# 12334zq/optical-flow-1

Hardware: AMD Instinct MI355X
Metric: Mpix*warp-iters/s, TV-L1 1920x1080 5-scale (higher is better)
Workload: dtype f64; 1 GPU; tvl1flow 1920x1080 pair (synthetic P1), nscales=5 warps=5 tau=0.25 lambda=0.15 theta=0.3 zfactor=0.5 epsilon=0.01; one pair per step per GPU; workload_name=1080p, arithmetic_mode=tolerance, pairs_per_gpu=1040, pairs_in_flight_per_gpu=64, lockstep_group=16, streams_per_gpu=4, distinct_pairs=8

## Files before the change

optical-flow-1_amd/csrc/ofx_device.h:

```cpp
#pragma once

#include <hip/hip_runtime.h>

#define OFX_DEV __device__ __forceinline__

OFX_DEV double  ldw(const double *p) { return *p; }
OFX_DEV double  ldw(const float *p)  { return (double) *p; }
OFX_DEV double2 ldw2(const double2 *p) { return *p; }
OFX_DEV double2 ldw2(const float2 *p)  { float2 v = *p; return make_double2((double) v.x, (double) v.y); }
OFX_DEV double4 ldw4(const double4 *p) { return *p; }
OFX_DEV double4 ldw4(const float4 *p)
{
    float4 v = *p;
    return make_double4((double) v.x, (double) v.y, (double) v.z, (double) v.w);
}
OFX_DEV void stn(double *p, double v) { *p = v; }
OFX_DEV void stn(float *p, double v)  { *p = (float) v; }
OFX_DEV void stn2(double2 *p, double2 v) { *p = v; }
OFX_DEV void stn2(float2 *p, double2 v)  { *p = make_float2((float) v.x, (float) v.y); }
typedef double ofx_d2v __attribute__((ext_vector_type(2)));
typedef float ofx_f2v __attribute__((ext_vector_type(2)));
OFX_DEV void stn2_nt(double2 *p, double2 v)
{
    ofx_d2v w;
    w.x = v.x; w.y = v.y;
    __builtin_nontemporal_store(w, reinterpret_cast<ofx_d2v *>(p));
}
OFX_DEV void stn2_nt(float2 *p, double2 v)
{
    ofx_f2v w;
    w.x = (float) v.x; w.y = (float) v.y;
    __builtin_nontemporal_store(w, reinterpret_cast<ofx_f2v *>(p));
}
template <bool NT, typename V> OFX_DEV void stn2_sel(V *p, double2 v)
{
    if (NT) stn2_nt(p, v);
    else stn2(p, v);
}
#define OFX_OOB 0xFFFFFFF0u
typedef unsigned ofx_u4v __attribute__((ext_vector_type(4)));
typedef unsigned ofx_u2v __attribute__((ext_vector_type(2)));
typedef __amdgpu_buffer_rsrc_t ofx_rsrc;
OFX_DEV ofx_rsrc make_rsrc(void *p, unsigned bytes) { return __builtin_amdgcn_make_buffer_rsrc(p, 0, bytes, 0x00020000); }
template <bool NT> OFX_DEV void bst2(ofx_rsrc r, unsigned byte_off, double2 v, const double2 *)
{
    ofx_u4v w;
    __builtin_memcpy(&w, &v, 16);
    __builtin_amdgcn_raw_buffer_store_b128(w, r, byte_off, 0, NT ? 2 : 0);
}
template <bool NT> OFX_DEV void bst2(ofx_rsrc r, unsigned byte_off, double2 v, const float2 *)
{
    const float2 f = make_float2((float) v.x, (float) v.y);
// ... 209 lines not shown
    }
    return cubic_cell(c[0], c[1], c[2], c[3], t.fx);
}

template <typename V2, typename S>
OFX_DEV void bicubic_sample3(const V2 *__restrict__ pa, const S *__restrict__ pb, const BicubicTaps &t, int nx,
                             double &o0, double &o1, double &o2)
{
    const unsigned E = sizeof(S);
    const unsigned r0 = (unsigned) t.row[0] * nx * E, r1 = (unsigned) t.row[1] * nx * E;
    const unsigned r2 = (unsigned) t.row[2] * nx * E, r3 = (unsigned) t.row[3] * nx * E;
    double c0[4], c1[4], c2[4];
#pragma unroll
    for (int k = 0; k < 4; k++) {
        const unsigned ck = (unsigned) t.col[k] * E;
        const char *ba = reinterpret_cast<const char *>(pa), *bb = reinterpret_cast<const char *>(pb);
        const double2 a0 = ldw2(reinterpret_cast<const V2 *>(ba + 2 * (r0 + ck)));
        const double2 a1 = ldw2(reinterpret_cast<const V2 *>(ba + 2 * (r1 + ck)));
        const double2 a2 = ldw2(reinterpret_cast<const V2 *>(ba + 2 * (r2 + ck)));
        const double2 a3 = ldw2(reinterpret_cast<const V2 *>(ba + 2 * (r3 + ck)));
        const double b0 = ldw(reinterpret_cast<const S *>(bb + r0 + ck));
        const double b1 = ldw(reinterpret_cast<const S *>(bb + r1 + ck));
        const double b2 = ldw(reinterpret_cast<const S *>(bb + r2 + ck));
        const double b3 = ldw(reinterpret_cast<const S *>(bb + r3 + ck));
        c0[k] = cubic_cell(a0.x, a1.x, a2.x, a3.x, t.fy);
        c1[k] = cubic_cell(a0.y, a1.y, a2.y, a3.y, t.fy);
        c2[k] = cubic_cell(b0, b1, b2, b3, t.fy);
    }
    o0 = cubic_cell(c0[0], c0[1], c0[2], c0[3], t.fx);
    o1 = cubic_cell(c1[0], c1[1], c1[2], c1[3], t.fx);
    o2 = cubic_cell(c2[0], c2[1], c2[2], c2[3], t.fx);
}

OFX_DEV double div_backward(double ac, double al, double bc, double bu, bool lef, bool rig, bool top, bool bot)
{
    if (!lef && !rig) {
        const double dxv = ac - al;
        return top ? dxv + bc : (bot ? dxv - bu : dxv + (bc - bu));
    }
    if (lef) return top ? ac + bc : (bot ? ac - bu : ac + bc - bu);
    return top ? -al + bc : (bot ? -al - bu : -al + bc - bu);
}
```

optical-flow-1_amd/csrc/ofx_ops.hip:

```cpp
#include "ofx_ops.h"
#include "ofx_device.h"

#include <cmath>

#define BX 64
#define BY 4

static inline dim3 grid2d(int nx, int ny) { return dim3(ofx_cdiv(nx, BX), ofx_cdiv(ny, BY)); }
static inline dim3 block2d() { return dim3(BX, BY); }
static inline int grid1d(size_t n) { return (int) ((n + 255) / 256); }

template <typename T>
__global__ void k_convert_in(const double *__restrict__ src, T *__restrict__ dst, size_t n)
{
    const size_t i = (size_t) blockIdx.x * blockDim.x + threadIdx.x;
    if (i < n) stn(dst + i, src[i]);
}

template <typename T>
__global__ void k_convert_out(const T *__restrict__ src, double *__restrict__ dst, size_t n)
{
    const size_t i = (size_t) blockIdx.x * blockDim.x + threadIdx.x;
    if (i < n) dst[i] = ldw(src + i);
}
// ... 253 lines not shown
    __shared__ double s_mid[(GXY_TH + 2 * GXY_RMAX) * 64];
    const T *__restrict__ in = in_p.at(blockIdx.z);
    T *__restrict__ out = out_p.at(blockIdx.z);
    const int R = taps.size - 1, W = 64 + 2 * R, H = GXY_TH + 2 * R;
    const int j0 = blockIdx.x * 64, i0 = blockIdx.y * GXY_TH;
    const int tid = threadIdx.y * 64 + threadIdx.x;
    for (int k = tid; k < W * H; k += 256) {
        const int r = k / W, c = k - r * W;
        int i = gauss_reflect(i0 - R + r, ny), j = gauss_reflect(j0 - R + c, nx);
        i = i < 0 ? 0 : (i > ny - 1 ? ny - 1 : i);
        j = j < 0 ? 0 : (j > nx - 1 ? nx - 1 : j);
        s_in[r * W + c] = ldw(in + (size_t) i * nx + j);
    }
    __syncthreads();
    for (int r = threadIdx.y; r < H; r += 4) {
        const double *row = s_in + r * W + R + threadIdx.x;
        double sum = taps.B[0] * row[0];
        for (int k = 1; k < taps.size; k++) sum += taps.B[k] * (row[-k] + row[k]);
        s_mid[r * 64 + threadIdx.x] = sizeof(T) == sizeof(float) ? (double) (float) sum : sum;
    }
    __syncthreads();
    const int j = j0 + threadIdx.x;
    if (j >= nx) return;
    for (int r = threadIdx.y; r < GXY_TH; r += 4) {
        const int i = i0 + r;
        if (i >= ny) break;
        const double *col = s_mid + (r + R) * 64 + threadIdx.x;
        double sum = taps.B[0] * col[0];
        for (int k = 1; k < taps.size; k++) sum += taps.B[k] * (col[-k * 64] + col[k * 64]);
        stn(out + (size_t) i * nx + j, sum);
    }
}

template <typename T, int R>
__global__ __launch_bounds__(256) void k_gauss_xy_gr(OfxPlanes2<const T> in_p, OfxPlanes2<T> out_p, int nx, int ny, GaussTaps taps)
{
    constexpr int W = 64 + 2 * R, H = GXY_TH + 2 * R;
    __shared__ double s_in[H * W];
    __shared__ double s_mid[H * 64];
    const T *__restrict__ in = in_p.at(blockIdx.z);
    T *__restrict__ out = out_p.at(blockIdx.z);
    const int j0 = blockIdx.x * 64, i0 = blockIdx.y * GXY_TH;
    const int tx = threadIdx.x, ty = threadIdx.y;
    int ja = gauss_reflect(j0 - R + tx, nx), jb = gauss_reflect(j0 - R + tx + 64, nx);
    ja = ja < 0 ? 0 : (ja > nx - 1 ? nx - 1 : ja);
    jb = jb < 0 ? 0 : (jb > nx - 1 ? nx - 1 : jb);
    for (int r = ty; r < H; r += 4) {
        int i = gauss_reflect(i0 - R + r, ny);
        i = i < 0 ? 0 : (i > ny - 1 ? ny - 1 : i);
        const T *__restrict__ row = in + (size_t) i * nx;
        s_in[r * W + tx] = ldw(row + ja);
        if (tx < 2 * R) s_in[r * W + tx + 64] = ldw(row + jb);
    }
    __syncthreads();
    for (int r = ty; r < H; r += 4) {
        const double *row = s_in + r * W + R + tx;
        double sum = taps.B[0] * row[0];
#pragma unroll
        for (int k = 1; k <= R; k++) sum += taps.B[k] * (row[-k] + row[k]);
        s_mid[r * 64 + tx] = sizeof(T) == sizeof(float) ? (double) (float) sum : sum;
    }
    __syncthreads();
    const int j = j0 + tx;
    if (j >= nx) return;
    constexpr int SEG = GXY_TH / 4;
    double win[SEG + 2 * R];
#pragma unroll
    for (int q = 0; q < SEG + 2 * R; q++) win[q] = s_mid[(ty * SEG + q) * 64 + tx];
#pragma unroll
    for (int o = 0; o < SEG; o++) {
        const int i = i0 + ty * SEG + o;
        double sum = taps.B[0] * win[o + R];
#pragma unroll
        for (int k = 1; k <= R; k++) sum += taps.B[k] * (win[o + R - k] + win[o + R + k]);
        if (i < ny) stn(out + (size_t) i * nx + j, sum);
    }
}
#define GXD_THO 12
template <typename T, int R>
__global__ __launch_bounds__(256) void k_gauss_xy_dec(OfxPlanes2<const T> in_p, OfxPlanes2<T> out_p, int nx, int ny, int nxo, int nyo,
                                                      GaussTaps taps)
{
    constexpr int W = 128 + 2 * R, H = 2 * GXD_THO + 2 * R;
    __shared__ double s_in[H * W];
    __shared__ double s_mid[H * 64];
    const T *__restrict__ in = in_p.at(blockIdx.z);
    T *__restrict__ out = out_p.at(blockIdx.z);
    const int j0 = blockIdx.x * 128, i0 = blockIdx.y * 2 * GXD_THO;
    const int tx = threadIdx.x, ty = threadIdx.y;
    int jc[3];
#pragma unroll
    for (int q = 0; q < 3; q++) {
        int j = gauss_reflect(j0 - R + tx + 64 * q, nx);
        jc[q] = j < 0 ? 0 : (j > nx - 1 ? nx - 1 : j);
    }
    for (int r = ty; r < H; r += 4) {
        int i = gauss_reflect(i0 - R + r, ny);
        i = i < 0 ? 0 : (i > ny - 1 ? ny - 1 : i);
        const T *__restrict__ row = in + (size_t) i * nx;
        s_in[r * W + tx] = ldw(row + jc[0]);
        s_in[r * W + tx + 64] = ldw(row + jc[1]);
        if (tx < 2 * R) s_in[r * W + tx + 128] = ldw(row + jc[2]);
    }
    __syncthreads();
    for (int r = ty; r < H; r += 4) {
        const double *row = s_in + r * W + R + 2 * tx;
        double sum = taps.B[0] * row[0];
#pragma unroll
        for (int k = 1; k <= R; k++) sum += taps.B[k] * (row[-k] + row[k]);
// ... 472 lines not shown
int op_build_pyramid_into(ofx_ctx *ctx, const T *dA, const T *dB, int nscales, double zfactor, double sigma,
                          const std::vector<ImgLevel<T>> &lv, T *tmpA, T *tmpB, double *scr)
{
    const int nxx = lv[0].nx, nyy = lv[0].ny;
    OFX_TRY(op_normalize2<T>(ctx, dA, dB, lv[0].A, lv[0].B, nxx * nyy, scr));
    OFX_TRY(op_gaussian<T>(ctx, lv[0].A, tmpA, nxx, nyy, sigma));
    OFX_TRY(op_gaussian<T>(ctx, lv[0].B, tmpA, nxx, nyy, sigma));
    for (int s = 1; s < nscales; s++) {
        OFX_TRY(op_zoom_out<T>(ctx, lv[s - 1].A, lv[s].A, tmpA, tmpB, lv[s - 1].nx, lv[s - 1].ny, zfactor));
        OFX_TRY(op_zoom_out<T>(ctx, lv[s - 1].B, lv[s].B, tmpA, tmpB, lv[s - 1].nx, lv[s - 1].ny, zfactor));
    }
    return OFX_OK;
}

template <typename T>
int op_build_pyramid_group(ofx_ctx *ctx, int G, const void *const *dA, const void *const *dB, int nscales, double zfactor,
                           double sigma, const int *nxs, const int *nys, T *const *lvA, T *const *lvB, T *tmpA, T *tmpB,
                           double *scr)
{
    if (G < 1 || G > OFX_MAX_GROUP) return ofx_fail(ctx, OFX_ERR_ARG, "pyramid group of %d", G);
    const int nxx = nxs[0], nyy = nys[0], size = nxx * nyy;
    OfxGroupPtrs P;
    for (int g = 0; g < OFX_MAX_GROUP; g++) { P.a[g] = g < G ? dA[g] : nullptr; P.b[g] = g < G ? dB[g] : nullptr; }
    int nb = grid1d((size_t) size);
    if (nb > MM_BLOCKS) nb = MM_BLOCKS;
    hipLaunchKernelGGL(k_minmax_partial_g<T>, dim3(nb, G), dim3(256), 0, ctx->stream, P, size, scr);
    OFX_LAUNCH_CHECK(ctx);
    hipLaunchKernelGGL(k_minmax_final_g, dim3(G), dim3(256), 0, ctx->stream, scr, nb);
    OFX_LAUNCH_CHECK(ctx);
    GaussTaps t0;
    const double zsigma = 0.6 * sqrt(1.0 / (zfactor * zfactor) - 1.0);
    bool fused = ctx->gauss_fused != 0 && ofx_gauss_taps(sigma, &t0) == OFX_OK && t0.size - 1 <= GXY_RMAX;
    if (fused && nscales > 1) fused = ofx_gauss_taps(zsigma, &t0) == OFX_OK && t0.size - 1 <= GXY_RMAX;
    T *n0 = fused ? tmpA : lvA[0], *n1 = fused ? tmpA + (size_t) G * size : lvB[0];
    hipLaunchKernelGGL(k_normalize2_g<T>, dim3(grid1d((size_t) size), G), dim3(256), 0, ctx->stream, P, n0, n1, size,
                       (const double *) scr);
    OFX_LAUNCH_CHECK(ctx);
    auto gauss_xy = [&](const T *ia, const T *ib, T *oa, T *ob, int nx, int ny, double sg) -> int {
        GaussTaps taps;
        if (ofx_gauss_taps(sg, &taps) != OFX_OK)
            return ofx_fail(ctx, OFX_ERR_ARG, "gaussian: sigma %g needs more than %d taps", sg, OFX_GAUSS_MAX_TAPS);
        if (taps.size >= nx || taps.size >= ny)
            return ofx_fail(ctx, OFX_ERR_SIGMA, "GaussianSmooth: sigma too large (radius %d, image %dx%d)", taps.size, nx, ny);
        const size_t st = (size_t) nx * ny;
        if (ctx->gauss_fused == 2)
            hipLaunchKernelGGL(k_gauss_xy_g<T>, dim3(ofx_cdiv(nx, 64), ofx_cdiv(ny, GXY_TH), 2 * G), dim3(64, 4), 0, ctx->stream,
                               OfxPlanes2<const T>{ia, ib, G, st}, OfxPlanes2<T>{oa, ob, G, st}, nx, ny, taps);
        else
            gauss_xy_launch<T>(ctx, dim3(ofx_cdiv(nx, 64), ofx_cdiv(ny, GXY_TH), 2 * G), OfxPlanes2<const T>{ia, ib, G, st},
                               OfxPlanes2<T>{oa, ob, G, st}, nx, ny, taps);
        OFX_LAUNCH_CHECK(ctx);
        return OFX_OK;
    };
    if (fused) {
        OFX_TRY(gauss_xy(n0, n1, lvA[0], lvB[0], nxx, nyy, sigma));
        for (int s = 1; s < nscales; s++) {
            const int nx = nxs[s - 1], ny = nys[s - 1];
            const size_t st = (size_t) nx * ny;
            GaussTaps tz;
            if (ctx->gauss_fused == 1 && zfactor == 0.5 && ofx_gauss_taps(zsigma, &tz) == OFX_OK && tz.size - 1 == 5 && tz.size < nx &&
                tz.size < ny && 2 * (nxs[s] - 1) <= nx - 1 && 2 * (nys[s] - 1) <= ny - 1) {
                hipLaunchKernelGGL((k_gauss_xy_dec<T, 5>), dim3(ofx_cdiv(nxs[s], 64), ofx_cdiv(nys[s], GXD_THO), 2 * G), dim3(64, 4), 0,
                                   ctx->stream, OfxPlanes2<const T>{lvA[s - 1], lvB[s - 1], G, st},
                                   OfxPlanes2<T>{lvA[s], lvB[s], G, (size_t) nxs[s] * nys[s]}, nx, ny, nxs[s], nys[s], tz);
                OFX_LAUNCH_CHECK(ctx);
                continue;
            }
            OFX_TRY(gauss_xy(lvA[s - 1], lvB[s - 1], tmpB, tmpB + (size_t) G * st, nx, ny, zsigma));
            dim3 g = grid2d(nxs[s], nys[s]);
            g.z = 2 * G;
            hipLaunchKernelGGL(k_resample_g<T>, g, block2d(), 0, ctx->stream, OfxPlanes2<const T>{tmpB, tmpB + (size_t) G * st, G, st},
                               OfxPlanes2<T>{lvA[s], lvB[s], G, (size_t) nxs[s] * nys[s]}, nx, ny, nxs[s], nys[s], zfactor, zfactor);
            OFX_LAUNCH_CHECK(ctx);
        }
        return OFX_OK;
    }
    auto gauss = [&](const T *ia, const T *ib, T *oa, T *ob, T *ta, T *tb, int nx, int ny, double sg) -> int {
        GaussTaps taps;
        if (ofx_gauss_taps(sg, &taps) != OFX_OK)
            return ofx_fail(ctx, OFX_ERR_ARG, "gaussian: sigma %g needs more than %d taps", sg, OFX_GAUSS_MAX_TAPS);
        if (taps.size >= nx || taps.size >= ny)
            return ofx_fail(ctx, OFX_ERR_SIGMA, "GaussianSmooth: sigma too large (radius %d, image %dx%d)", taps.size, nx, ny);
        const size_t st = (size_t) nx * ny;
        dim3 g = grid2d(nx, ny);
        g.z = 2 * G;
        hipLaunchKernelGGL((k_gauss_pass_g<T, true>), g, block2d(), 0, ctx->stream, OfxPlanes2<const T>{ia, ib, G, st},
                           OfxPlanes2<T>{ta, tb, G, st}, nx, ny, taps);
        OFX_LAUNCH_CHECK(ctx);
// ... 105 lines not shown
```

optical-flow-1_amd/csrc/ofx_sor.hip:

```cpp
#include "ofx_ops.h"
#include "ofx_device.h"
#include "ofx_loop.h"
#include "ofx_sor_tile.h"

#include <algorithm>

#include <atomic>
#include <cmath>
#include <new>
#include <thread>

#define HS_SOR_W 1.9
#define HS_PLANE_C_SKEW 2
#define BROX_PLANE_C_SKEW 1
#define HS_PRESMOOTH_SIGMA 0.8
#define BROX_EPSILON 0.001
#define BROX_SOR_W 1.9
#define BROX_SIGMA 0.8

template <typename T> OFX_DEV double rnd_to(double x);
template <> OFX_DEV double rnd_to<double>(double x) { return x; }
template <> OFX_DEV double rnd_to<float>(double x) { return (double) (float) x; }

static inline dim3 g2d(int nx, int ny) { return dim3(ofx_cdiv(nx, 64), ofx_cdiv(ny, 4)); }
static inline dim3 b2d() { return dim3(64, 4); }

static int sor_pick_chunk(const ofx_ctx *ctx, int nx, int ny, int launches_per_sweep)
{
    if (ctx->chunk > 0) return ctx->chunk;
    const double est_us = fmax(4.0 * launches_per_sweep, (double) nx * ny * 100.0 / 2.0e6);
    int c = (int) (60.0 / est_us);
    return c < 2 ? 2 : (c > 32 ? 32 : c);
}


template <typename T>
__global__ void k_hs_warp(const typename Pix<T>::v2 *__restrict__ pa, const T *__restrict__ pb, const T *__restrict__ I1,
                          const typename Pix<T>::v2 *__restrict__ U, const typename Pix<T>::v2 *__restrict__ U1, unsigned ucode,
                          typename Pix<T>::v2 *__restrict__ A, T *__restrict__ Dif, int nx, int ny)
{
    const int j = blockIdx.x * 64 + threadIdx.x;
    const int i = blockIdx.y * 4 + threadIdx.y;
    if (j >= nx || i >= ny) return;
    const size_t go = (size_t) blockIdx.z * nx * ny;
    if ((ucode >> blockIdx.z) & 1u) U = U1;
    pa += go; pb += go; I1 += go; U += go; A += go; Dif += go;
    const size_t p = (size_t) i * nx + j;
    const double2 u = ldw2(U + p);
    const BicubicTaps t = bicubic_taps(j + u.x, i + u.y, nx, ny);
    double I2w = 0.0, I2wx = 0.0, I2wy = 0.0;
    if (!t.out) {
        bicubic_sample3(pa, pb, t, nx, I2w, I2wx, I2wy);
        I2wx = rnd_to<T>(I2wx);
        I2wy = rnd_to<T>(I2wy);
    }
// ... 2808 lines not shown
```

optical-flow-1_amd/csrc/ofx_tvl1.hip:

```cpp
#include "ofx_ops.h"
#include "ofx_device.h"
#include "ofx_loop.h"

#include <atomic>
#include <chrono>
#include <cmath>
#include <thread>

#define TVL1_GRAD_IS_ZERO 1E-10
#define TVL1_PRESMOOTHING_SIGMA 0.8
#define STRIP_OUT 62

template <typename T> OFX_DEV double rnd_to(double x);
template <> OFX_DEV double rnd_to<double>(double x) { return x; }
template <> OFX_DEV double rnd_to<float>(double x) { return (double) (float) x; }

#ifdef OFX_NO_RFL
#define OFX_WAVE_UNIFORM(x) (x)
#else
#define OFX_WAVE_UNIFORM(x) __builtin_amdgcn_readfirstlane(x)
#endif
template <typename T> struct RowIn {
    double2 u, p1, p2, a;
    double r;
};

template <typename V> OFX_DEV const V *at(const V *base, unsigned byte_off)
{
    return reinterpret_cast<const V *>(reinterpret_cast<const char *>(base) + byte_off);
}
template <typename V> OFX_DEV V *at(V *base, unsigned byte_off)
{
    return reinterpret_cast<V *>(reinterpret_cast<char *>(base) + byte_off);
}

template <typename T>
OFX_DEV RowIn<T> tvl1_load_row(const typename Pix<T>::v2 *U, const typename Pix<T>::v2 *P1,
                               const typename Pix<T>::v2 *P2, const typename Pix<T>::v2 *A, const T *R, unsigned off2)
{
    RowIn<T> r;
    r.u = ldw2(at(U, off2));
    r.p1 = ldw2(at(P1, off2));
    r.p2 = ldw2(at(P2, off2));
    r.a = ldw2(at(A, off2));
    r.r = ldw(at(R, off2 >> 1));
    return r;
}

// ... 732 lines not shown
    const size_t goff = (size_t) g * nx * ny;
    const typename Pix<T>::v2 *__restrict__ pa = pag + goff;
    const T *__restrict__ pb = pbg + goff;
    const T *__restrict__ I0 = I0g + goff;
    const typename Pix<T>::v2 *__restrict__ U = pick3(Ut, curcode, g, (size_t) nx * ny).in;
    typename Pix<T>::v2 *__restrict__ A = Ag + goff;
    T *__restrict__ R = Rg + goff;
    const size_t p = (size_t) i * nx + j;
    const double2 u = ldw2(U + p);
    const BicubicTaps t = bicubic_taps(j + u.x, i + u.y, nx, ny);
    double I1w = 0.0, I1wx = 0.0, I1wy = 0.0;
    if (!t.out) {
        bicubic_sample3(pa, pb, t, nx, I1w, I1wx, I1wy);
        I1wx = rnd_to<T>(I1wx);
        I1wy = rnd_to<T>(I1wy);
    }
    stn2(A + p, make_double2(I1wx, I1wy));
    stn(R + p, (I1w - I1wx * u.x - I1wy * u.y - ldw(I0 + p)));
}

#ifndef WARP_TW
#define WARP_TW 48
#define WARP_TH 16
#endif
#ifndef WARP_BY
#define WARP_BY 8
#endif
#ifndef WARP_WAVES
#define WARP_WAVES 8
#endif
#define WARP_ATTR __attribute__((amdgpu_waves_per_eu(WARP_WAVES, WARP_WAVES)))
#define WARP_NT (32 * WARP_BY)
#define WARP_NW (WARP_NT / 64)
template <typename T>
__global__ __launch_bounds__(WARP_NT) WARP_ATTR void k_tvl1_warp_lds(
    const typename Pix<T>::v2 *__restrict__ pag, const T *__restrict__ pbg, const T *__restrict__ I0g,
    Tri<typename Pix<T>::v2> Ut, typename Pix<T>::v2 *__restrict__ Ag, T *__restrict__ Rg, int nx, int ny,
    unsigned curcode)
{
    __shared__ double2 s_a[WARP_TH * WARP_TW];
    __shared__ double s_b[WARP_TH * WARP_TW];
    __shared__ int s_box[WARP_NW][4];
    const int tid = threadIdx.y * 32 + threadIdx.x, wave = tid >> 6;
    const int j = blockIdx.x * 32 + threadIdx.x;
    const int i = blockIdx.y * WARP_BY + threadIdx.y;
    const bool inside = (j < nx) && (i < ny);
    const int g = blockIdx.z;
    const size_t goff = (size_t) g * nx * ny;
    const typename Pix<T>::v2 *__restrict__ pa = pag + goff;
    const T *__restrict__ pb = pbg + goff;
    const typename Pix<T>::v2 *__restrict__ U = pick3(Ut, curcode, g, (size_t) nx * ny).in;
    const size_t p = (size_t) (inside ? i : 0) * nx + (inside ? j : 0);
    double2 u = make_double2(0.0, 0.0);
    BicubicTaps t;
    t.out = true;
    if (inside) {
        u = ldw2(U + p);
        t = bicubic_taps(j + u.x, i + u.y, nx, ny);
    }
    const bool need = inside && !t.out;
    int xlo = need ? t.col[0] : 0x7fffffff, xhi = need ? t.col[3] : -1;
    int ylo = need ? t.row[0] : 0x7fffffff, yhi = need ? t.row[3] : -1;
#pragma unroll
    for (int m = 32; m >= 1; m >>= 1) {
        xlo = min(xlo, __shfl_xor(xlo, m, 64)); xhi = max(xhi, __shfl_xor(xhi, m, 64));
        ylo = min(ylo, __shfl_xor(ylo, m, 64)); yhi = max(yhi, __shfl_xor(yhi, m, 64));
    }
    if ((tid & 63) == 0) { s_box[wave][0] = xlo; s_box[wave][1] = xhi; s_box[wave][2] = ylo; s_box[wave][3] = yhi; }
    __syncthreads();
#pragma unroll
    for (int w = 0; w < WARP_NW; w++) {
        xlo = min(xlo, s_box[w][0]); xhi = max(xhi, s_box[w][1]);
        ylo = min(ylo, s_box[w][2]); yhi = max(yhi, s_box[w][3]);
    }
    const int W = xhi - xlo + 1, H = yhi - ylo + 1;
    const bool any = (xhi >= 0);
    const bool tile = any && W <= WARP_TW && H <= WARP_TH;
    if (tile) {
        for (int k = tid; k < W * H; k += WARP_NT) {
            const int r = k / W, c = k - r * W;
            const size_t src = (size_t) (ylo + r) * nx + (xlo + c);
            s_a[r * WARP_TW + c] = ldw2(pa + src);
            s_b[r * WARP_TW + c] = ldw(pb + src);
        }
        __syncthreads();
    }
    if (!inside) return;
    double I1w = 0.0, I1wx = 0.0, I1wy = 0.0;
    if (need) {
        if (tile) {
            const int cx = t.col[0] - xlo, cy = t.row[0] - ylo;
            double c0[4], c1[4], c2[4];
#pragma unroll
            for (int k = 0; k < 4; k++) {
                const int o = cy * WARP_TW + cx + k;
                const double2 a0 = s_a[o], a1 = s_a[o + WARP_TW], a2 = s_a[o + 2 * WARP_TW], a3 = s_a[o + 3 * WARP_TW];
                const double b0 = s_b[o], b1 = s_b[o + WARP_TW], b2 = s_b[o + 2 * WARP_TW], b3 = s_b[o + 3 * WARP_TW];
                c0[k] = cubic_cell(a0.x, a1.x, a2.x, a3.x, t.fy);
                c1[k] = cubic_cell(a0.y, a1.y, a2.y, a3.y, t.fy);
                c2[k] = cubic_cell(b0, b1, b2, b3, t.fy);
            }
            I1w = cubic_cell(c0[0], c0[1], c0[2], c0[3], t.fx);
            I1wx = cubic_cell(c1[0], c1[1], c1[2], c1[3], t.fx);
            I1wy = cubic_cell(c2[0], c2[1], c2[2], c2[3], t.fx);
        } else {
            bicubic_sample3(pa, pb, t, nx, I1w, I1wx, I1wy);
        }
        I1wx = rnd_to<T>(I1wx);
        I1wy = rnd_to<T>(I1wy);
    }
    stn2(Ag + goff + p, make_double2(I1wx, I1wy));
    stn(Rg + goff + p, (I1w - I1wx * u.x - I1wy * u.y - ldw(I0g + goff + p)));
}

template <typename T>
__global__ void k_tvl1_zoom_in_g(Tri<typename Pix<T>::v2> Ut, unsigned curcode, typename Pix<T>::v2 *__restrict__ Uout, int nx,
                                 int ny, int nxx, int nyy, double fx, double fy, double scale)
{
    const int j1 = blockIdx.x * 64 + threadIdx.x;
    const int i1 = blockIdx.y * 4 + threadIdx.y;
    if (j1 >= nxx || i1 >= nyy) return;
    const int g = blockIdx.z;
    const typename Pix<T>::v2 *__restrict__ U = pick3(Ut, curcode, g, (size_t) nx * ny).in;
    const double i2 = i1 / fy, j2 = j1 / fx;
    const BicubicTaps t = bicubic_taps(j2, i2, nx, ny);
    double c1[4], c2[4];
#pragma unroll
    for (int k = 0; k < 4; k++) {
        const double2 v0 = ldw2(U + (size_t) t.row[0] * nx + t.col[k]);
        const double2 v1 = ldw2(U + (size_t) t.row[1] * nx + t.col[k]);
        const double2 v2 = ldw2(U + (size_t) t.row[2] * nx + t.col[k]);
        const double2 v3 = ldw2(U + (size_t) t.row[3] * nx + t.col[k]);
        c1[k] = cubic_cell(v0.x, v1.x, v2.x, v3.x, t.fy);
        c2[k] = cubic_cell(v0.y, v1.y, v2.y, v3.y, t.fy);
    }
    double2 r;
    r.x = cubic_cell(c1[0], c1[1], c1[2], c1[3], t.fx) * scale;
    r.y = cubic_cell(c2[0], c2[1], c2[2], c2[3], t.fx) * scale;
    stn2(Uout + (size_t) g * nxx * nyy + (size_t) i1 * nxx + j1, r);
}

template <typename T>
__global__ void k_tvl1_to_flo_g(Tri<typename Pix<T>::v2> Ut, unsigned curcode, OfxGroupPtrs out, size_t n)
{
    const size_t i = (size_t) blockIdx.x * blockDim.x + threadIdx.x;
// ... 13 lines not shown
    v2 *U[3], *P1[3], *P2[3], *A;
    T  *R;
    unsigned cur;
    int last_n[OFX_MAX_GROUP];
    size_t n() const { return (size_t) nx * ny; }
    unsigned curidx(int g) const { return (cur >> (2 * g)) & 3u; }
    v2 *Ucur(int g) const { return U[curidx(g)] + (size_t) g * n(); }
    v2 *P1cur(int g) const { return P1[curidx(g)] + (size_t) g * n(); }
    v2 *P2cur(int g) const { return P2[curidx(g)] + (size_t) g * n(); }
    Tri<v2> Ut() const { return Tri<v2>{U[0], U[1], U[2]}; }
    Tri<v2> P1t() const { return Tri<v2>{P1[0], P1[1], P1[2]}; }
    Tri<v2> P2t() const { return Tri<v2>{P2[0], P2[1], P2[2]}; }
};

struct Tvl1Params {
    double tau, lambda, theta, epsilon;
    int warps, verbose, max_iter;
    bool fixed;
};

template <typename T> static int tvl1_level_alloc(ofx_ctx *ctx, Tvl1Level<T> &L, int nx, int ny, int G, bool images)
{
    const size_t n = (size_t) nx * ny * G;
    L.nx = nx;
    L.ny = ny;
    L.G = G;
    L.cur = 0;
    for (int g = 0; g < OFX_MAX_GROUP; g++) L.last_n[g] = 0;
    L.I0 = L.I1 = nullptr;
    if (images) {
        OFX_TRY(ofx_alloc(ctx, n, &L.I0));
        OFX_TRY(ofx_alloc(ctx, n, &L.I1));
    }
    OFX_TRY(ofx_alloc(ctx, n, &L.pa));
    OFX_TRY(ofx_alloc(ctx, n, &L.pb));
    for (int h = 0; h < 3; h++) {
        OFX_TRY(ofx_alloc(ctx, n, &L.U[h]));
        OFX_TRY(ofx_alloc(ctx, n, &L.P1[h]));
        OFX_TRY(ofx_alloc(ctx, n, &L.P2[h]));
    }
    OFX_TRY(ofx_alloc(ctx, n, &L.A));
    OFX_TRY(ofx_alloc(ctx, n, &L.R));
    return OFX_OK;
}

static int tvl1_pick_rows(const ofx_ctx *ctx, int nx, int ny, int G)
{
    if (ctx->rows_per_wave > 0) return ctx->rows_per_wave;
    const long strips = (long) ofx_cdiv(nx, STRIP_OUT) * G;
    if (strips * ofx_cdiv(ny, 4) >= 2048) return 4;
    if (strips * ofx_cdiv(ny, 2) >= 1024) return 2;
    return 1;
}

static int tvl1_pick_rows2(const ofx_ctx *ctx, int nx, int ny, int G)
{
    if (ctx->rows_per_wave2 > 0) return ctx->rows_per_wave2;
    const long strips_pad = (long) ofx_cdiv(ofx_cdiv(nx, STRIP2_OUT), 4) * 4 * G;
    const int rmax = 24;
    int best = rmax;
    long best_cost = -1;
    if (ctx->concurrency > 1) {
        static const int cand[] = {1, 2, 3, 4, 5, 6, 8, 10, 12, 14, 16, 20, 24};
        for (int r : cand) {
            const long waves = strips_pad * ofx_cdiv(ny, r);
            const long slots = ctx->rows_slots > 0 ? ctx->rows_slots : 1024;
            const long cost = ((waves + slots - 1) / slots) * (r + 5);
            if (best_cost < 0 || cost < best_cost) { best_cost = cost; best = r; }
// ... 311 lines not shown
                const int n = k_of[g] + 1, j = (n - 1) / 3;
                runmask |= 1u << g;
                incode |= ((b0[g] + (unsigned) j) % 3u) << (2 * g);
                nit |= (unsigned long long) (n - j * 3) << (4 * g);
            }
            return go(0, 0, S.max_iter, -1.0, incode, runmask, nit, nullptr, 0);
        };
        int took_alt[OFX_MAX_GROUP];
        OFX_TRY(ofx_run_loop_group(ctx, S, G, launch, redo, n_out, err_out, ms_out, 0u, took_alt));
        for (int g = 0; g < G; g++) {
            unit_of[g] = n_out[g] > 0 ? (n_out[g] - 1) / 3 : -1;
            inside[g] = (n_out[g] % 3 != 0 && n_out[g] != S.max_iter) ? 1 : 0;
        }
    }
    unsigned cur = 0;
    for (int g = 0; g < G; g++) {
        const unsigned units = (unsigned) (unit_of[g] + 1);
        cur |= ((b0[g] + units) % 3u) << (2 * g);
        L.last_n[g] = n_out[g];
        if (alt_out) alt_out[g] = inside[g] ? 1 : 0;
    }
    L.cur = cur;
    return OFX_OK;
}

template <typename T>
static int tvl1_single_scale_dev(ofx_ctx *ctx, Tvl1Level<T> &L, const Tvl1Params &P, int scale, ofx_stats *stats)
{
    const int nx = L.nx, ny = L.ny, G = L.G;
    const size_t n = L.n();
    const dim3 g2(ofx_cdiv(nx, OFX_WARP_BX), ofx_cdiv(ny, OFX_WARP_BY), G), b2(OFX_WARP_BX, OFX_WARP_BY);
    if (nx < 2 || ny < 2) return ofx_fail(ctx, OFX_ERR_ARG, "tvl1: level %dx%d too small", nx, ny);

    OFX_TRY(op_grad_pack<T>(ctx, L.I1, L.pa, L.pb, nx, ny, G));
    for (int h = 0; h < 3; h++) {
        bool used = false;
        for (int g = 0; g < G; g++) used = used || (L.curidx(g) == (unsigned) h);
        if (!used) continue;
        OFX_TRY(op_fill2<T>(ctx, L.P1[h], n * G));
        OFX_TRY(op_fill2<T>(ctx, L.P2[h], n * G));
    }
    for (int g = 0; g < G; g++) L.last_n[g] = 0;

    for (int w = 0; w < P.warps; w++) {
        if (ctx->warp_lds)
            hipLaunchKernelGGL(k_tvl1_warp_lds<T>, dim3(ofx_cdiv(nx, 32), ofx_cdiv(ny, WARP_BY), G), dim3(32, WARP_BY), 0, ctx->stream, L.pa,
                               (const T *) L.pb, (const T *) L.I0, L.Ut(), L.A, L.R, nx, ny, L.cur);
        else
            hipLaunchKernelGGL(k_tvl1_warp<T>, g2, b2, 0, ctx->stream, L.pa, (const T *) L.pb, (const T *) L.I0, L.Ut(),
                               L.A, L.R, nx, ny, L.cur);
        OFX_LAUNCH_CHECK(ctx);
        int it[OFX_MAX_GROUP];
        double error[OFX_MAX_GROUP];
        float ms = 0.f;
        int odd[OFX_MAX_GROUP], unit = 0;
        OFX_TRY(tvl1_run_iterations<T>(ctx, L, P, it, error, ctx->profile ? &ms : nullptr, odd, &unit));
        if (P.verbose && G == 1) fprintf(stderr, "Warping: %d, Iterations: %d, Error: %f\n", w, it[0], error[0]);
        for (int g = 0; g < G; g++) {
            ofx_stats &S = stats[g];
            S.odd_stops += odd[g] != 0;
            S.odd_stops_stored += odd[g] == 2;
            if (scale < OFX_MAX_SCALES) {
                S.fused[scale] = unit;
                if (w < OFX_MAX_SOLVES) { S.iters[scale][w] = it[g]; S.error[scale][w] = error[g]; }
                S.iter_ms[scale] += ms;
                S.iter_launches[scale] += it[g];
            }
            S.work_pix_iters += (double) it[g] * nx * ny;
        }
    }
    return OFX_OK;
}

static void stats_begin(ofx_stats *st, int nscales, int nsolves)
{
    memset(st, 0, sizeof(*st));
    st->nscales = nscales;
    st->nsolves = nsolves;
}

// ... 430 lines not shown
```

Measured before the change: 79820 Mpix*warp-iters/s.

## Compute I1 gradients on the fly in warp kernel and fuse normalize into Gaussian

The LDS warp kernel now loads a haloed tile of the raw I1 image and computes the central-difference gradients inside the bicubic sampling. This removes the separate grad_pack pass and the packed gradient buffers, and it reduces the bytes loaded per tile. The pyramid build also folds min/max normalization into the first fused Gaussian's load, which drops a full-resolution normalize kernel and its intermediate write. The cost is extra arithmetic and LDS reads per sample, plus a slower fallback sampler outside the tile that does more global loads.

```diff
diff --git a/optical-flow-1_amd/csrc/ofx_device.h b/optical-flow-1_amd/csrc/ofx_device.h
--- a/optical-flow-1_amd/csrc/ofx_device.h
+++ b/optical-flow-1_amd/csrc/ofx_device.h
@@ -18,6 +18,9 @@
 OFX_DEV void stn(float *p, double v)  { *p = (float) v; }
 OFX_DEV void stn2(double2 *p, double2 v) { *p = v; }
 OFX_DEV void stn2(float2 *p, double2 v)  { *p = make_float2((float) v.x, (float) v.y); }
+template <typename T> OFX_DEV double rnd_to(double x);
+template <> OFX_DEV double rnd_to<double>(double x) { return x; }
+template <> OFX_DEV double rnd_to<float>(double x) { return (double) (float) x; }
 typedef double ofx_d2v __attribute__((ext_vector_type(2)));
 typedef float ofx_f2v __attribute__((ext_vector_type(2)));
 OFX_DEV void stn2_nt(double2 *p, double2 v)
@@ -293,6 +296,36 @@
     o2 = cubic_cell(c2[0], c2[1], c2[2], c2[3], t.fx);
 }
 
+template <typename T>
+OFX_DEV void bicubic_sample3(const T *__restrict__ f, const BicubicTaps &t, int nx, int ny, double &o0, double &o1, double &o2)
+{
+    double c0[4] = {0.0, 0.0, 0.0, 0.0}, c1[4] = {0.0, 0.0, 0.0, 0.0}, c2[4] = {0.0, 0.0, 0.0, 0.0};
+    const int sx = t.col[2] - t.col[1], sy = t.row[2] - t.row[1];
+#pragma unroll 1
+    for (int k = 0; k < 4; k++) {
+        const int j = t.col[1] + (k - 1) * sx, jl = j > 0 ? j - 1 : 0, jr = j < nx - 1 ? j + 1 : nx - 1;
+        double v[4] = {0.0, 0.0, 0.0, 0.0}, vx[4] = {0.0, 0.0, 0.0, 0.0}, vy[4] = {0.0, 0.0, 0.0, 0.0};
+#pragma unroll 1
+        for (int m = 0; m < 4; m++) {
+            const int i = t.row[1] + (m - 1) * sy, iu = i > 0 ? i - 1 : 0, id = i < ny - 1 ? i + 1 : ny - 1;
+            const T *__restrict__ row = f + (size_t) i * nx;
+#pragma unroll
+            for (int q = 0; q < 3; q++) { v[q] = v[q + 1]; vx[q] = vx[q + 1]; vy[q] = vy[q + 1]; }
+            v[3] = ldw(row + j);
+            vx[3] = rnd_to<T>(0.5 * (ldw(row + jr) - ldw(row + jl)));
+            vy[3] = rnd_to<T>(0.5 * (ldw(f + (size_t) id * nx + j) - ldw(f + (size_t) iu * nx + j)));
+        }
+#pragma unroll
+        for (int q = 0; q < 3; q++) { c0[q] = c0[q + 1]; c1[q] = c1[q + 1]; c2[q] = c2[q + 1]; }
+        c0[3] = cubic_cell(v[0], v[1], v[2], v[3], t.fy);
+        c1[3] = cubic_cell(vx[0], vx[1], vx[2], vx[3], t.fy);
+        c2[3] = cubic_cell(vy[0], vy[1], vy[2], vy[3], t.fy);
+    }
+    o0 = cubic_cell(c0[0], c0[1], c0[2], c0[3], t.fx);
+    o1 = cubic_cell(c1[0], c1[1], c1[2], c1[3], t.fx);
+    o2 = cubic_cell(c2[0], c2[1], c2[2], c2[3], t.fx);
+}
+
 OFX_DEV double div_backward(double ac, double al, double bc, double bu, bool lef, bool rig, bool top, bool bot)
 {
     if (!lef && !rig) {
diff --git a/optical-flow-1_amd/csrc/ofx_ops.hip b/optical-flow-1_amd/csrc/ofx_ops.hip
--- a/optical-flow-1_amd/csrc/ofx_ops.hip
+++ b/optical-flow-1_amd/csrc/ofx_ops.hip
@@ -309,14 +309,25 @@
     }
 }
 
-template <typename T, int R>
-__global__ __launch_bounds__(256) void k_gauss_xy_gr(OfxPlanes2<const T> in_p, OfxPlanes2<T> out_p, int nx, int ny, GaussTaps taps)
+template <typename T> struct GaussLoadPlane {
+    const T *__restrict__ in;
+    OFX_DEV double operator()(size_t o) const { return ldw(in + o); }
+};
+template <typename T> struct GaussLoadNorm2 {
+    const T *__restrict__ in;
+    double lo, den;
+    OFX_DEV double operator()(size_t o) const
+    {
+        const double a = ldw(in + o);
+        return den > 0 ? rnd_to<T>(255.0 * (a - lo) / den) : a;
+    }
+};
+template <typename T, int R, typename Ld>
+OFX_DEV void gauss_xy_r_block(const Ld ld, T *__restrict__ out, int nx, int ny, const GaussTaps &taps)
 {
     constexpr int W = 64 + 2 * R, H = GXY_TH + 2 * R;
     __shared__ double s_in[H * W];
     __shared__ double s_mid[H * 64];
-    const T *__restrict__ in = in_p.at(blockIdx.z);
-    T *__restrict__ out = out_p.at(blockIdx.z);
     const int j0 = blockIdx.x * 64, i0 = blockIdx.y * GXY_TH;
     const int tx = threadIdx.x, ty = threadIdx.y;
     int ja = gauss_reflect(j0 - R + tx, nx), jb = gauss_reflect(j0 - R + tx + 64, nx);
@@ -325,9 +336,9 @@
     for (int r = ty; r < H; r += 4) {
         int i = gauss_reflect(i0 - R + r, ny);
         i = i < 0 ? 0 : (i > ny - 1 ? ny - 1 : i);
-        const T *__restrict__ row = in + (size_t) i * nx;
-        s_in[r * W + tx] = ldw(row + ja);
-        if (tx < 2 * R) s_in[r * W + tx + 64] = ldw(row + jb);
+        const size_t row = (size_t) i * nx;
+        s_in[r * W + tx] = ld(row + ja);
+        if (tx < 2 * R) s_in[r * W + tx + 64] = ld(row + jb);
     }
     __syncthreads();
     for (int r = ty; r < H; r += 4) {
@@ -352,6 +363,20 @@
         for (int k = 1; k <= R; k++) sum += taps.B[k] * (win[o + R - k] + win[o + R + k]);
         if (i < ny) stn(out + (size_t) i * nx + j, sum);
     }
+}
+template <typename T, int R>
+__global__ __launch_bounds__(256) void k_gauss_xy_gr(OfxPlanes2<const T> in_p, OfxPlanes2<T> out_p, int nx, int ny, GaussTaps taps)
+{
+    gauss_xy_r_block<T, R>(GaussLoadPlane<T>{in_p.at(blockIdx.z)}, out_p.at(blockIdx.z), nx, ny, taps);
+}
+template <typename T, int R>
+__global__ __launch_bounds__(256) void k_gauss_xy_gr_norm(OfxGroupPtrs P, int G, const double *__restrict__ scr, OfxPlanes2<T> out_p,
+                                                          int nx, int ny, GaussTaps taps)
+{
+    const int z = blockIdx.z, g = z < G ? z : z - G;
+    const double *__restrict__ mm = scr + (size_t) g * MM_SCR + 2 * MM_BLOCKS;
+    const double lo = mm[0], den = mm[1] - mm[0];
+    gauss_xy_r_block<T, R>(GaussLoadNorm2<T>{(const T *) (z < G ? P.a[g] : P.b[g]), lo, den}, out_p.at(z), nx, ny, taps);
 }
 #define GXD_THO 12
 template <typename T, int R>
@@ -890,10 +915,15 @@
     const double zsigma = 0.6 * sqrt(1.0 / (zfactor * zfactor) - 1.0);
     bool fused = ctx->gauss_fused != 0 && ofx_gauss_taps(sigma, &t0) == OFX_OK && t0.size - 1 <= GXY_RMAX;
     if (fused && nscales > 1) fused = ofx_gauss_taps(zsigma, &t0) == OFX_OK && t0.size - 1 <= GXY_RMAX;
+    GaussTaps ts;
+    const bool norm_on_load = fused && ctx->gauss_fused == 1 && ofx_gauss_taps(sigma, &ts) == OFX_OK && ts.size - 1 >= 1 &&
+                              ts.size < nxx && ts.size < nyy;
     T *n0 = fused ? tmpA : lvA[0], *n1 = fused ? tmpA + (size_t) G * size : lvB[0];
-    hipLaunchKernelGGL(k_normalize2_g<T>, dim3(grid1d((size_t) size), G), dim3(256), 0, ctx->stream, P, n0, n1, size,
-                       (const double *) scr);
-    OFX_LAUNCH_CHECK(ctx);
+    if (!norm_on_load) {
+        hipLaunchKernelGGL(k_normalize2_g<T>, dim3(grid1d((size_t) size), G), dim3(256), 0, ctx->stream, P, n0, n1, size,
+                           (const double *) scr);
+        OFX_LAUNCH_CHECK(ctx);
+    }
     auto gauss_xy = [&](const T *ia, const T *ib, T *oa, T *ob, int nx, int ny, double sg) -> int {
         GaussTaps taps;
         if (ofx_gauss_taps(sg, &taps) != OFX_OK)
@@ -911,7 +941,18 @@
         return OFX_OK;
     };
     if (fused) {
-        OFX_TRY(gauss_xy(n0, n1, lvA[0], lvB[0], nxx, nyy, sigma));
+        if (norm_on_load) {
+            const dim3 grid(ofx_cdiv(nxx, 64), ofx_cdiv(nyy, GXY_TH), 2 * G);
+            const OfxPlanes2<T> out{lvA[0], lvB[0], G, (size_t) size};
+#define OFX_GXYN(R_) case R_: hipLaunchKernelGGL((k_gauss_xy_gr_norm<T, R_>), grid, dim3(64, 4), 0, ctx->stream, P, G, (const double *) scr, out, nxx, nyy, ts); break
+            switch (ts.size - 1) {
+                OFX_GXYN(1); OFX_GXYN(2); OFX_GXYN(3); OFX_GXYN(4); OFX_GXYN(5); OFX_GXYN(6); OFX_GXYN(7); OFX_GXYN(8);
+            }
+#undef OFX_GXYN
+            OFX_LAUNCH_CHECK(ctx);
+        } else {
+            OFX_TRY(gauss_xy(n0, n1, lvA[0], lvB[0], nxx, nyy, sigma));
+        }
         for (int s = 1; s < nscales; s++) {
             const int nx = nxs[s - 1], ny = nys[s - 1];
             const size_t st = (size_t) nx * ny;
diff --git a/optical-flow-1_amd/csrc/ofx_sor.hip b/optical-flow-1_amd/csrc/ofx_sor.hip
--- a/optical-flow-1_amd/csrc/ofx_sor.hip
+++ b/optical-flow-1_amd/csrc/ofx_sor.hip
@@ -18,9 +18,6 @@
 #define BROX_SOR_W 1.9
 #define BROX_SIGMA 0.8
 
-template <typename T> OFX_DEV double rnd_to(double x);
-template <> OFX_DEV double rnd_to<double>(double x) { return x; }
-template <> OFX_DEV double rnd_to<float>(double x) { return (double) (float) x; }
 
 static inline dim3 g2d(int nx, int ny) { return dim3(ofx_cdiv(nx, 64), ofx_cdiv(ny, 4)); }
 static inline dim3 b2d() { return dim3(64, 4); }
diff --git a/optical-flow-1_amd/csrc/ofx_tvl1.hip b/optical-flow-1_amd/csrc/ofx_tvl1.hip
--- a/optical-flow-1_amd/csrc/ofx_tvl1.hip
+++ b/optical-flow-1_amd/csrc/ofx_tvl1.hip
@@ -11,9 +11,6 @@
 #define TVL1_PRESMOOTHING_SIGMA 0.8
 #define STRIP_OUT 62
 
-template <typename T> OFX_DEV double rnd_to(double x);
-template <> OFX_DEV double rnd_to<double>(double x) { return x; }
-template <> OFX_DEV double rnd_to<float>(double x) { return (double) (float) x; }
 
 #ifdef OFX_NO_RFL
 #define OFX_WAVE_UNIFORM(x) (x)
@@ -812,14 +809,13 @@
 #define WARP_ATTR __attribute__((amdgpu_waves_per_eu(WARP_WAVES, WARP_WAVES)))
 #define WARP_NT (32 * WARP_BY)
 #define WARP_NW (WARP_NT / 64)
+#define WARP_SW (WARP_TW + 2)
 template <typename T>
 __global__ __launch_bounds__(WARP_NT) WARP_ATTR void k_tvl1_warp_lds(
-    const typename Pix<T>::v2 *__restrict__ pag, const T *__restrict__ pbg, const T *__restrict__ I0g,
-    Tri<typename Pix<T>::v2> Ut, typename Pix<T>::v2 *__restrict__ Ag, T *__restrict__ Rg, int nx, int ny,
-    unsigned curcode)
-{
-    __shared__ double2 s_a[WARP_TH * WARP_TW];
-    __shared__ double s_b[WARP_TH * WARP_TW];
+    const T *__restrict__ I1g, const T *__restrict__ I0g, Tri<typename Pix<T>::v2> Ut, typename Pix<T>::v2 *__restrict__ Ag,
+    T *__restrict__ Rg, int nx, int ny, unsigned curcode)
+{
+    __shared__ double s_i[(WARP_TH + 2) * WARP_SW];
     __shared__ int s_box[WARP_NW][4];
     const int tid = threadIdx.y * 32 + threadIdx.x, wave = tid >> 6;
     const int j = blockIdx.x * 32 + threadIdx.x;
@@ -827,15 +823,16 @@
     const bool inside = (j < nx) && (i < ny);
     const int g = blockIdx.z;
     const size_t goff = (size_t) g * nx * ny;
-    const typename Pix<T>::v2 *__restrict__ pa = pag + goff;
-    const T *__restrict__ pb = pbg + goff;
+    const T *__restrict__ I1 = I1g + goff;
     const typename Pix<T>::v2 *__restrict__ U = pick3(Ut, curcode, g, (size_t) nx * ny).in;
     const size_t p = (size_t) (inside ? i : 0) * nx + (inside ? j : 0);
     double2 u = make_double2(0.0, 0.0);
     BicubicTaps t;
     t.out = true;
+    double i0 = 0.0;
     if (inside) {
         u = ldw2(U + p);
+        i0 = ldw(I0g + goff + p);
         t = bicubic_taps(j + u.x, i + u.y, nx, ny);
     }
     const bool need = inside && !t.out;
@@ -857,11 +854,20 @@
     const bool any = (xhi >= 0);
     const bool tile = any && W <= WARP_TW && H <= WARP_TH;
     if (tile) {
-        for (int k = tid; k < W * H; k += WARP_NT) {
-            const int r = k / W, c = k - r * W;
-            const size_t src = (size_t) (ylo + r) * nx + (xlo + c);
-            s_a[r * WARP_TW + c] = ldw2(pa + src);
-            s_b[r * WARP_TW + c] = ldw(pb + src);
+        constexpr int RP = WARP_NT / 64, NP = (WARP_TH + 2 + RP - 1) / RP;
+        static_assert(WARP_SW <= 64, "a tile row is loaded by one wave");
+        const int c = tid & 63, r0 = tid >> 6;
+        const int x = min(max(xlo - 1 + c, 0), nx - 1);
+        double v[NP];
+#pragma unroll
+        for (int q = 0; q < NP; q++) {
+            const int r = r0 + q * RP, y = min(max(ylo - 1 + r, 0), ny - 1);
+            if (c < W + 2 && r < H + 2) v[q] = ldw(I1 + (size_t) y * nx + x);
+        }
+#pragma unroll
+        for (int q = 0; q < NP; q++) {
+            const int r = r0 + q * RP;
+            if (c < W + 2 && r < H + 2) s_i[r * WARP_SW + c] = v[q];
         }
         __syncthreads();
     }
@@ -869,28 +875,46 @@
     double I1w = 0.0, I1wx = 0.0, I1wy = 0.0;
     if (need) {
         if (tile) {
-            const int cx = t.col[0] - xlo, cy = t.row[0] - ylo;
+            const double *s = s_i + (t.row[0] - ylo + 1) * WARP_SW + (t.col[0] - xlo + 1);
             double c0[4], c1[4], c2[4];
 #pragma unroll
             for (int k = 0; k < 4; k++) {
-                const int o = cy * WARP_TW + cx + k;
-                const double2 a0 = s_a[o], a1 = s_a[o + WARP_TW], a2 = s_a[o + 2 * WARP_TW], a3 = s_a[o + 3 * WARP_TW];
-                const double b0 = s_b[o], b1 = s_b[o + WARP_TW], b2 = s_b[o + 2 * WARP_TW], b3 = s_b[o + 3 * WARP_TW];
-                c0[k] = cubic_cell(a0.x, a1.x, a2.x, a3.x, t.fy);
-                c1[k] = cubic_cell(a0.y, a1.y, a2.y, a3.y, t.fy);
-                c2[k] = cubic_cell(b0, b1, b2, b3, t.fy);
+                double c[6], vy[4];
+#pragma unroll
+                for (int q = 0; q < 6; q++) c[q] = s[(q - 1) * WARP_SW + k];
+#pragma unroll
+                for (int m = 0; m < 4; m++) vy[m] = rnd_to<T>(0.5 * (c[m + 2] - c[m]));
+                c0[k] = cubic_cell(c[1], c[2], c[3], c[4], t.fy);
+                c2[k] = cubic_cell(vy[0], vy[1], vy[2], vy[3], t.fy);
+                __builtin_amdgcn_sched_barrier(0);
+            }
+            double l[4], c[4], r[4];
+#pragma unroll
+            for (int m = 0; m < 4; m++) { l[m] = s[m * WARP_SW - 1]; c[m] = s[m * WARP_SW]; }
+#pragma unroll
+            for (int k = 0; k < 4; k++) {
+                double vx[4];
+#pragma unroll
+                for (int m = 0; m < 4; m++) {
+                    r[m] = s[m * WARP_SW + k + 1];
+                    vx[m] = rnd_to<T>(0.5 * (r[m] - l[m]));
+                    l[m] = c[m];
+                    c[m] = r[m];
+                }
+                c1[k] = cubic_cell(vx[0], vx[1], vx[2], vx[3], t.fy);
+                __builtin_amdgcn_sched_barrier(0);
             }
             I1w = cubic_cell(c0[0], c0[1], c0[2], c0[3], t.fx);
             I1wx = cubic_cell(c1[0], c1[1], c1[2], c1[3], t.fx);
             I1wy = cubic_cell(c2[0], c2[1], c2[2], c2[3], t.fx);
         } else {
-            bicubic_sample3(pa, pb, t, nx, I1w, I1wx, I1wy);
+            bicubic_sample3<T>(I1, t, nx, ny, I1w, I1wx, I1wy);
         }
         I1wx = rnd_to<T>(I1wx);
         I1wy = rnd_to<T>(I1wy);
     }
     stn2(Ag + goff + p, make_double2(I1wx, I1wy));
-    stn(Rg + goff + p, (I1w - I1wx * u.x - I1wy * u.y - ldw(I0g + goff + p)));
+    stn(Rg + goff + p, (I1w - I1wx * u.x - I1wy * u.y - i0));
 }
 
 template <typename T>
@@ -970,8 +994,12 @@
         OFX_TRY(ofx_alloc(ctx, n, &L.I0));
         OFX_TRY(ofx_alloc(ctx, n, &L.I1));
     }
-    OFX_TRY(ofx_alloc(ctx, n, &L.pa));
-    OFX_TRY(ofx_alloc(ctx, n, &L.pb));
+    L.pa = nullptr;
+    L.pb = nullptr;
+    if (!ctx->warp_lds) {
+        OFX_TRY(ofx_alloc(ctx, n, &L.pa));
+        OFX_TRY(ofx_alloc(ctx, n, &L.pb));
+    }
     for (int h = 0; h < 3; h++) {
         OFX_TRY(ofx_alloc(ctx, n, &L.U[h]));
         OFX_TRY(ofx_alloc(ctx, n, &L.P1[h]));
@@ -1349,7 +1377,7 @@
     const dim3 g2(ofx_cdiv(nx, OFX_WARP_BX), ofx_cdiv(ny, OFX_WARP_BY), G), b2(OFX_WARP_BX, OFX_WARP_BY);
     if (nx < 2 || ny < 2) return ofx_fail(ctx, OFX_ERR_ARG, "tvl1: level %dx%d too small", nx, ny);
 
-    OFX_TRY(op_grad_pack<T>(ctx, L.I1, L.pa, L.pb, nx, ny, G));
+    if (!ctx->warp_lds) OFX_TRY(op_grad_pack<T>(ctx, L.I1, L.pa, L.pb, nx, ny, G));
     for (int h = 0; h < 3; h++) {
         bool used = false;
         for (int g = 0; g < G; g++) used = used || (L.curidx(g) == (unsigned) h);
@@ -1361,8 +1389,8 @@
 
     for (int w = 0; w < P.warps; w++) {
         if (ctx->warp_lds)
-            hipLaunchKernelGGL(k_tvl1_warp_lds<T>, dim3(ofx_cdiv(nx, 32), ofx_cdiv(ny, WARP_BY), G), dim3(32, WARP_BY), 0, ctx->stream, L.pa,
-                               (const T *) L.pb, (const T *) L.I0, L.Ut(), L.A, L.R, nx, ny, L.cur);
+            hipLaunchKernelGGL(k_tvl1_warp_lds<T>, dim3(ofx_cdiv(nx, 32), ofx_cdiv(ny, WARP_BY), G), dim3(32, WARP_BY), 0, ctx->stream,
+                               (const T *) L.I1, (const T *) L.I0, L.Ut(), L.A, L.R, nx, ny, L.cur);
         else
             hipLaunchKernelGGL(k_tvl1_warp<T>, g2, b2, 0, ctx->stream, L.pa, (const T *) L.pb, (const T *) L.I0, L.Ut(),
                                L.A, L.R, nx, ny, L.cur);
```

Result: faster. 80700 Mpix*warp-iters/s (median of 6 runs) (+1.1%).
